# ogotoh/prrn_aln

Hardware: AMD Instinct MI355X
Metric: DP cells/s (profile-profile fwd2) + SP-score delta vs ref, 256x1024aa refinement (higher is better)
Workload: dtype f64; 1 GPU; prrn refinement sweep: 256 proteins x 1024 aa (seed 1), start MSA 5459 columns, 509 tree-branch divisions (HLF/RHF 256, GPF 253), 2.986e+09 in-band cells/sweep, band sh=-60; divisions=509, parallelism=divisions round-robin by size over 1 GPU(s), skeleton_corners=895772

## Files before the change

prrn_aln_amd/csrc/g2g_kernels.hip:

```cpp
#include <hip/hip_runtime.h>
#include <float.h>
#include <limits.h>
#include "g2g_device.h"

#define NEVSEL (-(DBL_MAX / 16 * 7))
#ifndef G2G_FWD_THREADS
#define G2G_FWD_THREADS 256
#endif
#ifndef G2G_V2_THREADS
#define G2G_V2_THREADS 256
#endif
#ifndef G2G_V2_MINWAVES
#define G2G_V2_MINWAVES 4
#endif
#ifndef G2G_V2_TILE_COLS
#define G2G_V2_TILE_COLS 256
#endif

enum { D_DEAD = 0, D_DIAG = 2, D_NEWD = 3, D_VERT = 4, D_HORI = 8, D_NEWV = 12, D_NEWH = 13 };
__device__ __forceinline__ bool isdiag(int d) { return d == D_DIAG || d == D_NEWD; }
__device__ __forceinline__ bool isvert(int d) { return d == D_VERT || d == D_NEWV; }
__device__ __forceinline__ bool ishori(int d) { return d == D_HORI || d == D_NEWH; }

enum { T_DIRMASK = 7, T_SEL2 = 8, T_GEXT = 16, T_G2EXT = 32, T_FEXT = 64, T_F2EXT = 128 };
// ... 61 lines not shown
    int k = 0;
    for (int di = 0; df.glen[di] >= 0; ++di) {
        while (df.glen[di] >= dld.glen(k + 1)) ++k;
        if (i < df.glen[di] + dld.nins(k)) break;
        g += df.freq[di];
    }
    return g;
}
__device__ __forceinline__ void cleardelta(const DList d) { d.set(0, 0, 0); d.set(1, INT_MAX, 0); }
__device__ void copydelta(const DList dst, const DList src)
{
    int k = 0;
    do { dst.set(k, src.glen(k), src.nins(k)); ++k; } while (src.glen(k) < INT_MAX);
    dst.set(k, src.glen(k), src.nins(k));
}
__device__ void newdelta(const DList dst, const SList df, const DList src)
{
    int kd = 0, ks = 0;
    int tg = 0, tn = 0;
    for (int di = 0; df.glen[di] >= 0; ++di) {
        int g = df.glen[di];
        if (g >= src.glen(ks)) {
            while (g >= src.glen(ks + 1)) ++ks;
            int sn = src.nins(ks);
            if (sn > tn) {
                dst.set(kd++, tg, tn);
                tn = sn;
                tg = g + 1;
            }
        }
    }
    dst.set(kd++, tg, tn);
    dst.set(kd, INT_MAX, 0);
}
__device__ void incdelta2(const DList dst, const DList src)
{
    int k = 0;
    do { dst.set(k, src.glen(k), src.nins(k) + 1); ++k; } while (src.glen(k) < INT_MAX);
    dst.set(k, src.glen(k), src.nins(k));
}

__device__ double sim2(const DevProb &P, int m, int n)
{
    const DevSide &a = P.a, &b = P.b;
    const uint8_t *ar = res_at(a, m), *br = res_at(b, n);
    const double *mtx = P.simmtx;
    const int dim = P.simdim;
    double s = 0;
    switch (P.sim2_kind) {
    case 0: return 0;
    case 11: return mtx[(size_t) ar[0] * dim + br[0]];
    case 120: for (int j = 0; j < b.many; ++j) s += mtx[(size_t) ar[0] * dim + br[j]]; return s;
    case 121: for (int j = 0; j < b.many; ++j) s += mtx[(size_t) ar[0] * dim + br[j]] * b.weight[j]; return s;
    case 13: return vss_at(b, n)[b.felm + ar[0]];
    case 210: for (int i = 0; i < a.many; ++i) s += mtx[(size_t) br[0] * dim + ar[i]]; return s;
    case 211: for (int i = 0; i < a.many; ++i) s += mtx[(size_t) br[0] * dim + ar[i]] * a.weight[i]; return s;
    case 220:
        for (int i = 0; i < a.many; ++i)
            for (int j = 0; j < b.many; ++j) s += mtx[(size_t) ar[i] * dim + br[j]];
        return s;
    case 221:
        for (int i = 0; i < a.many; ++i) {
            double st = 0;
            for (int j = 0; j < b.many; ++j) st += mtx[(size_t) ar[i] * dim + br[j]] * b.weight[j];
            s += st * a.weight[i];
        }
        return s;
    case 230: { const double *vb = vss_at(b, n) + b.felm;
        for (int i = 0; i < a.many; ++i) s += vb[ar[i]]; return s; }
    case 231: { const double *vb = vss_at(b, n) + b.felm;
        for (int i = 0; i < a.many; ++i) s += vb[ar[i]] * a.weight[i]; return s; }
    case 31: return vss_at(a, m)[a.felm + br[0]];
    case 320: { const double *va = vss_at(a, m) + a.felm;
        for (int j = 0; j < b.many; ++j) s += va[br[j]]; return s; }
    case 321: { const double *va = vss_at(a, m) + a.felm;
        for (int j = 0; j < b.many; ++j) s += va[br[j]] * b.weight[j]; return s; }
    case 33: { const double *va = vss_at(a, m) + a.felm, *vb = vss_at(b, n);
        for (int j = 0; j < b.felm; ++j) s += va[j] * vb[j]; return s; }
    case 330: { const double *va = vss_at(a, m) + a.felm, *vb = vss_at(b, n);
        const int dc[6] = {0, 1, 2, 3, 5, 9};
        for (int j = 0; j < b.felm; ++j) s += va[dc[j]] * vb[j]; return s; }
    }
    return 0;
}

__device__ __forceinline__ double unpa(const DevProb &P, int m, int n) { return thk_at(P.a, m)[0] * thk_at(P.b, n)[2] * -P.u; }
__device__ __forceinline__ double unpb(const DevProb &P, int n, int m) { return thk_at(P.b, n)[0] * thk_at(P.a, m)[2] * -P.u; }

__device__ double crg2(const DevProb &P, const int *gla, const int *glb, int st, int m, int n, int d3)
{
    const DevSide &a = P.a, &b = P.b;
    const uint8_t *as = res_at(a, m), *bs = res_at(b, n);
    const double *agd = a.gapdens + (size_t)(m + 1) * a.many, *apg = a.postgapdens + (size_t)(m + 1) * a.many;
    const double *bgd = b.gapdens + (size_t)(n + 1) * b.many, *bpg = b.postgapdens + (size_t)(n + 1) * b.many;
    const double *wa = a.weight, *wb = b.weight;
    const int an = a.many, bn = b.many;
#define GLA(i) gla[(size_t)(i) * st]
#define GLB(j) glb[(size_t)(j) * st]
#define NG(c) ((c) > 1)
    double g = 0;
    switch (P.crg2_kind) {
    case 11:
        if (d3 == 0) {
            if (NG(as[0]) && bgd[0] > 0 && GLA(0) >= GLB(0)) return bgd[0] * P.basic_gop;
            if (NG(bs[0]) && agd[0] > 0 && GLB(0) >= GLA(0)) return agd[0] * P.basic_gop;
        } else if (d3 > 0) {
            if (bpg[0] > 0 && GLA(0) >= GLB(0)) return bpg[0] * P.basic_gop;
        } else {
            if (apg[0] > 0 && GLB(0) >= GLA(0)) return apg[0] * P.basic_gop;
        }
        return 0;
    case 120: case 121: {
        const bool w = P.crg2_kind & 1;
        if (d3 == 0) {
            if (NG(as[0])) {
                for (int j = 0; j < bn; ++j) if (bgd[j] > 0 && GLA(0) >= GLB(j)) g += w ? wb[j] * bgd[j] : bgd[j];
            } else if (agd[0] > 0) {
                for (int j = 0; j < bn; ++j) if (NG(bs[j]) && GLB(j) >= GLA(0)) g += w ? wb[j] * agd[0] : agd[0];
            }
        } else if (d3 > 0) {
            if (NG(as[0]))
                for (int j = 0; j < bn; ++j) if (bpg[j] > 0 && GLA(0) >= GLB(j)) g += w ? wb[j] * bpg[j] : bpg[j];
        } else if (apg[0] > 0) {
            for (int j = 0; j < bn; ++j) if (NG(bs[j]) && GLB(j) >= GLA(0)) g += w ? wb[j] * apg[0] : apg[0];
        }
        return g * P.basic_gop;
    }
    case 210: case 211: {
        const bool w = P.crg2_kind & 1;
        if (d3 == 0) {
            if (NG(bs[0])) {
                for (int i = 0; i < an; ++i) if (agd[i] > 0 && GLB(0) >= GLA(i)) g += w ? wa[i] * agd[i] : agd[i];
            } else if (bgd[0] > 0) {
                for (int i = 0; i < an; ++i) if (NG(as[i]) && GLA(i) >= GLB(0)) g += w ? wa[i] * bgd[0] : bgd[0];
            }
        } else if (d3 < 0) {
            if (NG(bs[0]))
                for (int i = 0; i < an; ++i) if (apg[i] > 0 && GLB(0) >= GLA(i)) g += w ? wa[i] * apg[i] : apg[i];
        } else if (!w || (bs[0] && bs[1])) {
            if (bpg[0] > 0)
                for (int i = 0; i < an; ++i) if (NG(as[i]) && GLA(i) >= GLB(0)) g += w ? wa[i] * bpg[0] : bpg[0];
        }
        return g * P.basic_gop;
    }
    case 220:
        if (d3 == 0) {
            for (int i = 0; i < an; ++i) {
                if (NG(as[i])) {
                    for (int j = 0; j < bn; ++j) if (bgd[j] > 0 && GLA(i) >= GLB(j)) g += bgd[j];
                } else if (agd[i] > 0) {
                    for (int j = 0; j < bn; ++j) if (NG(bs[j]) && GLB(j) >= GLA(i)) g += agd[i];
                }
            }
        } else if (d3 > 0) {
            for (int i = 0; i < an; ++i)
                if (NG(as[i]))
                    for (int j = 0; j < bn; ++j) if (bpg[j] > 0 && GLA(i) >= GLB(j)) g += bpg[j];
        } else {
            for (int j = 0; j < bn; ++j)
                if (NG(bs[j]))
                    for (int i = 0; i < an; ++i) if (apg[i] > 0 && GLB(j) >= GLA(i)) g += apg[i];
        }
        return g * P.basic_gop;
    case 221:
        if (d3 == 0) {
            for (int i = 0; i < an; ++i) {
// ... 1342 lines not shown
```

prrn_aln_amd/csrc/g2g_kernels_v6.hip:

```cpp
#include <hip/hip_runtime.h>

#ifdef G2G_V6_STAMP
__device__ unsigned long long g2g_v6_stamp_acc[16];
#define V6_STAMP(k) { const unsigned long long t_ = __builtin_amdgcn_s_memtime(); st_acc[k] += t_ - st_t; st_t = t_; }
#define V6_STAMP_ARGS , unsigned long long (&st_acc)[12], unsigned long long &st_t
#define V6_STAMP_PASS , st_acc, st_t
#else
#define V6_STAMP(k)
#define V6_STAMP_ARGS
#define V6_STAMP_PASS
#endif

#include "g2g_lds.h"

struct LS6 { const lu32 *rows0; GLB unsigned *tw; int ia, ib; };
__device__ __forceinline__ GLB unsigned *ls6_twin(const LS6 &W, const lu32 *p, const int k) { return W.tw + 2 * (int) (p - W.rows0) + k; }
__device__ __forceinline__ unsigned ls6_rd(const LS6 &W, const lu32 *p, const int k, const int I) { return k < I ? p[k] : *ls6_twin(W, p, k); }
__device__ __forceinline__ void ls6_wr(const LS6 &W, lu32 *p, const int k, const int I, const unsigned v)
{
    if (k < I) p[k] = v;
    else { *ls6_twin(W, p, k) = v; asm volatile("s_waitcnt vmcnt(0)" ::: "memory"); }
}

#define V6_UNROLL _Pragma("clang loop unroll(full)")
// ... 472 lines not shown
            const GLB double *bfr = glb(b.freq[v]);
            lu32 *rk = (lu32 *) (lds + LO.ringk[v]);
            lf64 *rf = (lf64 *) (lds + LO.ringf[v]);
            const int S = v == 0 ? RS0 : RS1, base = v == 0 ? rbase0 : rbase1;
            for (int c0_ = fedcol + 1; c0_ <= upto; c0_ += 64) {
                const int col = c0_ + lane;
                if (col <= upto) {
                    const int k0 = bo[col + 1], len = bo[col + 2] - k0 - 1, c = k0 - (col + 1);
                    for (int e = 0; e < len; ++e) {
                        const int i = v6_ring_slot(c + e, base, S);
                        const unsigned key = v6_key(bgl[k0 + e]);
                        const double f = bfr[k0 + e];
                        rk[i] = key; rf[i] = f;
                        if (i < RT) { rk[S + i] = key; rf[S + i] = f; }
                    }
                }
            }
        }
        {
            const GLB double *bfr2 = glb(b.freq[2]);
            for (int c0_ = fedcol + 1; c0_ <= upto; c0_ += 64) {
                const int col = c0_ + lane;
                if (col <= upto) {
                    const int k2 = boff2[col + 1], lr_ = boff2[col + 2] - k2 - 1, lt_ = boff1[col + 2] - boff1[col + 1] - 1;
                    rhring[col & (V6_RHCOLS - 1)] = lr_ > lt_ ? bfr2[k2] : -1.;
                }
            }
        }
        if (upto > fedcol) fedcol = upto;
    };
    RS oH = rs_black(), oG = rs_black(), oG2 = rs_black(), oF = rs_black(), oF2 = rs_black();
    if (row_ok && m + 1 < a.right && m + 1 <= m_left_last && m + 1 + P.lw <= b.left) {
        lu32 *p = V6_L(lane + 1, SLOT_H(c0));
        const GLB unsigned *src = colH + (size_t) (m + 1 - a.left) * ndw;
        oH.val = __hiloint2double((int) V6_XLD(src + 1), (int) V6_XLD(src)); oH.dir = (int) V6_XLD(src + 2); oH.glb = (int) V6_XLD(src + 3);
        for (int k = 0; k < capa; ++k) { const unsigned v = V6_XLD(src + 4 + k); ls6_wr(W, p, k, ca4, v); if (v >= TERM) break; }
        for (int k = 0; k < capb; ++k) { const unsigned v = V6_XLD(src + 4 + capa + k); ls6_wr(W, p + ca4, k, cb4, v); if (v >= TERM) break; }
    }
    auto stage_load = [&](int col, bool wantG, unsigned &rh, unsigned &rg, unsigned &rg2) {
        if (lane < ndw) {
            const GLB unsigned *s = (col == b.left && vert0) ? colH + (size_t) (m0 - a.left) * ndw : rowHp + (size_t) col * ndw;
            rh = V6_XLD(s + lane);
            if (wantG) { rg = V6_XLD(rowGp + (size_t) col * ndw + lane); if (NOLL3) rg2 = V6_XLD(rowG2p + (size_t) col * ndw + lane); }
        }
    };
    auto stage_put = [&](int slot, int sid, unsigned v) {
        const int j = lane - 4;
        lu32 *const p = V6_L(0, slot);
        if (lane < 4) stsc[sid * 4 + lane] = v;
        else if (j < ca4 && j < capa) p[j] = v;
        else if (j >= capa && j - capa < cb4 && j < capa + capb) p[ca4 + j - capa] = v;
        if (capa > ca4 || capb > cb4) {
            const unsigned long long tb = __ballot(v >= TERM) >> 4;
            const int ta = tb ? (int) __builtin_ctzll(tb) : 63;
            const unsigned long long tbb = capa < 60 ? tb >> capa : 0ull;
            const int tbp = tbb ? (int) __builtin_ctzll(tbb) : 63;
            if (j >= ca4 && j < capa && j <= ta) ls6_wr(W, p, j, ca4, v);
            if (j >= capa + cb4 && j < capa + capb && j - capa <= tbp) ls6_wr(W, p + ca4, j - capa, cb4, v);
        }
    };
    auto stage_store = [&](int col, bool wantG, unsigned rh, unsigned rg, unsigned rg2) {
        if (lane < ndw) {
            stage_put(SLOT_H(col), SLOT_H(col), rh);
            if (wantG) { stage_put(SLOT_G(col), 3 + (col & 1), rg); if (NOLL3) stage_put(SLOT_G2(col), 5 + (col & 1), rg2); }
        }
    };
    StripSync S = strip_sync(prog_up, prog_self, dbg, failp, pgen, ti);
    if (lane < 28) stsc[lane] = 0;
    team_sync();
    refill(cbase);
    strip_need<V6Strip>(S, cbase + 1 <= c1 ? cbase + 1 : cbase);
    {
        unsigned rh = 0, rg = 0, rg2 = 0;
        stage_load(cbase, false, rh, rg, rg2);
        stage_store(cbase, false, rh, rg, rg2);
        if (cbase + 1 <= c1) {
            stage_load(cbase + 1, vert0, rh, rg, rg2);
            stage_store(cbase + 1, vert0, rh, rg, rg2);
        }
    }
    const double a_efq = row_ok ? thk_at(a, m)[2] : 0;
    const double pua_row = row_ok ? unpa(P, m, nlo) : 0;
    SimBlk SB; SB.buf = (GLBV3 double *) simscr; SB.cbase = cbase;
    simblk_fill(P, SB, 0, m0, lane);
    asm volatile("s_waitcnt vmcnt(0)" ::: "memory");
    double sim_cur = 0, bc_cur = 0;
    int os_cur = 0, oe_cur = 0, ot_cur = 0, te_cur = 0;
    bool have = false;
    RS hu = rs_black(), gu = rs_black(), g2u = rs_black(), hd;
    const bool do_vert = m > a.left;
    const bool wr_rows = mend < a.right;
    team_sync();
    unsigned st_h = 0, st_g = 0, st_g2 = 0;
    bool st_prev = false;
    bool p_act = false; int p_trb = 0; size_t p_tri = 0;
    const int ull = __builtin_amdgcn_readfirstlane(llast);
    int lhi = m0 + llast + P.up + 1; if (lhi > b.right) lhi = b.right;
    int llo = m0 + llast + P.lw; if (llo < b.left) llo = b.left;
    auto flush_rows = [&](const int nl) {
        if (nl >= llo && nl < lhi) {
            const int col = nl + 1;
            const int j = lane - 4;
#pragma unroll
            for (int x = 0; x < (NOLL3 ? 3 : 2); ++x) {
                const RS &r = (x == 0) ? oH : (x == 1) ? oG : oG2;
                const int slot = (x == 0) ? SLOT_H(col) : (x == 1) ? SLOT_G(col) : SLOT_G2(col);
                const unsigned v0 = (unsigned) __builtin_amdgcn_readlane(__double2loint(r.val), ull);
                const unsigned v1 = (unsigned) __builtin_amdgcn_readlane(__double2hiint(r.val), ull);
                const unsigned v2 = (unsigned) __builtin_amdgcn_readlane(r.dir, ull), v3 = (unsigned) __builtin_amdgcn_readlane(r.glb, ull);
                unsigned v = lane == 0 ? v0 : lane == 1 ? v1 : lane == 2 ? v2 : v3;
                if (lane >= 4 && lane < ndw) {
                    const lu32 *p = V6_L(llast + 1, slot);
                    v = (j < capa) ? (j < ca4 ? p[j] : TERM) : (j < capa + capb) ? (j - capa < cb4 ? p[ca4 + j - capa] : TERM) : 0;
                    if (capa > ca4 && p[ca4 - 1] < TERM && j >= ca4 && j < capa) v = ls6_rd(W, p, j, ca4);
                    if (capb > cb4 && p[ca4 + cb4 - 1] < TERM && j >= capa + cb4 && j < capa + capb) v = ls6_rd(W, p + ca4, j - capa, cb4);
                }
                GLB unsigned *dst = (x == 0) ? rowHc : (x == 1) ? rowGc : rowG2c;
                if (lane < ndw) V6_XST(dst + (size_t) col * ndw + lane, v);
            }
        }
    };
#ifdef G2G_V6_STAMP
    unsigned long long st_acc[12] = {0, 0, 0, 0, 0, 0, 0, 0, 0, 0, 0, 0};
    unsigned long long st_t = __builtin_amdgcn_s_memtime();
#endif
    strip_where(S);
    for (int s = 0; s < nsteps; ++s) {
        V6_STAMP(9)
        V6_BEAT(s)
        V6_MARK(1)
        const int n = cbase + s - lane;
        const int n0 = cbase + s;
        const bool active = row_ok && n >= lo && n < hi;
        if (st_prev) stage_store(n0 + 1, vert0, st_h, st_g, st_g2);
        if (p_act) trace[p_tri] = (uint8_t) p_trb;
        if (wr_rows && s > 0) flush_rows(n0 - 1 - llast);
        if (prog_self && s > 0 && (s & (pint - 1)) == 0) strip_publish<V6Strip>(S, n0 - llast);
        if ((s & (V6_FEED - 1)) == 0) { V6_MARK(2) refill(n0); team_sync(); }
        if ((s & 63) == 0) { V6_MARK(3) simblk_fill(P, SB, (s >> 6) + 1, m0, lane); asm volatile("s_waitcnt vmcnt(0)" ::: "memory"); }
        hd = hu;
        hu = rs_up(oH); gu = rs_up(oG);
        if (NOLL3) g2u = rs_up(oG2);
        strip_handover<V6Strip, NOLL3>(stsc, n0, lane, hd, hu, gu, g2u);
        double sim_nx = 0, bc_nx = 0;
        int os_nx = 0, oe_nx = 0, ot_nx = 0, te_nx = 0;
        if (active) {
            if (!have) {
                sim_cur = *simblk_at(SB, lane, n); bc_cur = bthk[(size_t) (n + 1) * 3];
                os_cur = boff0[n + 1]; oe_cur = boff0[n + 2]; ot_cur = boff1[n + 1]; te_cur = boff1[n + 2];
            }
            if (n + 1 < hi) {
                sim_nx = *simblk_at(SB, lane, n + 1); bc_nx = bthk[(size_t) (n + 2) * 3];
                os_nx = oe_cur; oe_nx = boff0[n + 3]; ot_nx = te_cur; te_nx = boff1[n + 3];
            }
        }
        st_prev = n0 + 1 < hi0 && n0 + 2 <= c1;
        if (st_prev) { V6_MARK(4) strip_need<V6Strip>(S, n0 + 2); stage_load(n0 + 2, vert0, st_h, st_g, st_g2); }
        V6_MARK(5)
        RS myH = oH, myG = oG, myG2 = oG2;
        V6_STAMP(0)
        if (active) {
            const bool do_hori = n > b.left;
            B6 B;
            B.rs = ring[0]; B.rt = ring[1];
            B.os = v6_ring_slot(os_cur - (n + 1), rbase0, RS0); B.ot = v6_ring_slot(ot_cur - (n + 1), rbase1, RS1);
            B.lens = oe_cur - os_cur - 1; B.lent = te_cur - ot_cur - 1;
            { const double hv = rhring[n & (V6_RHCOLS - 1)]; B.rhf = hv >= 0 ? hv : 0.; B.lenr = B.lent + (hv >= 0 ? 1 : 0); }
            const bool up_in = do_vert && (n - (m - 1) <= P.up);
            const bool left_in = (n - 1 - m >= P.lw);
            const RS bk = rs_black();
            const RS s_hu = rs_sel(up_in, hu, bk), s_gu = rs_sel(up_in, gu, bk), s_g2u = rs_sel(up_in, g2u, bk);
            const RS s_hl = rs_sel(left_in, oH, bk), s_fl = rs_sel(left_in, oF, bk), s_f2l = rs_sel(left_in, oF2, bk);
            const lu32 *hdl = V6_L(lane, SLOT_H(n));
            const lu32 *hul = up_in ? V6_L(lane, SLOT_H(n + 1)) : blk;
            const lu32 *gul = up_in ? V6_L(lane, SLOT_G(n + 1)) : blk;
            const lu32 *g2ul = (NOLL3 && up_in) ? V6_L(lane, SLOT_G2(n + 1)) : blk;
            const lu32 *hll = left_in ? V6_L(lane + 1, SLOT_H(n)) : blk;
            const lu32 *fll = left_in ? V6_L(lane + 1, SLOT_F) : blk;
            const lu32 *f2ll = (NOLL3 && left_in) ? V6_L(lane + 1, SLOT_F2) : blk;
            lu32 *const sink = (lu32 *) (lds + LO.sink) + lane;
            lu32 *const sink16 = (lu32 *) (lds + LO.sink) + 64 + 4 * lane;
            lu32 *dh = V6_L(lane + 1, SLOT_H(n + 1));
            lu32 *dg = V6_L(lane + 1, SLOT_G(n + 1));
            lu32 *dg2 = V6_L(lane + 1, NOLL3 ? SLOT_G2(n + 1) : SLOT_G(n + 1));
            lu32 *df = V6_L(lane + 1, SLOT_F);
            lu32 *df2 = V6_L(lane + 1, NOLL3 ? SLOT_F2 : SLOT_F);
            const double pua = a.nils ? unpa(P, m, n) : pua_row;
            const double pub = bc_cur * a_efq * -P.u;
            int trb = 0;
            if (!v6_cell_pf<NOLL3, NA, 5, false>(P, W, A, TAs, TAt, B, sink, sink16, hd, hdl, s_hu, hul, s_gu, gul, s_g2u, g2ul, s_hl, hll, s_fl, fll, s_f2l, f2ll,
                                  dh, dg, dg2, df, df2, do_vert, do_hori, sim_cur, pua, pub, myH, myG, myG2, oF, oF2, trb V6_STAMP_PASS))
                if (!v6_cell_pf<NOLL3, NA, 8, false>(P, W, A, TAs, TAt, B, sink, sink16, hd, hdl, s_hu, hul, s_gu, gul, s_g2u, g2ul, s_hl, hll, s_fl, fll, s_f2l, f2ll,
                                  dh, dg, dg2, df, df2, do_vert, do_hori, sim_cur, pua, pub, myH, myG, myG2, oF, oF2, trb V6_STAMP_PASS))
                    v6_cell_pf<NOLL3, NA, 8, true>(P, W, A, TAs, TAt, B, sink, sink16, hd, hdl, s_hu, hul, s_gu, gul, s_g2u, g2ul, s_hl, hll, s_fl, fll, s_f2l, f2ll,
                                  dh, dg, dg2, df, df2, do_vert, do_hori, sim_cur, pua, pub, myH, myG, myG2, oF, oF2, trb V6_STAMP_PASS);
            const int d = m + n;
            int mlo, mhi;
            diag_rows(d, a.left, a.right, b.left, b.right, P.lw, P.up, &mlo, &mhi);
            p_tri = (size_t) (d - P.d0) * P.tstride + (m - mlo);
            p_trb = trb;
            sim_cur = sim_nx; bc_cur = bc_nx; have = (n + 1 < hi);
            os_cur = os_nx; oe_cur = oe_nx; ot_cur = ot_nx; te_cur = te_nx;
            if (m == a.right - 1 && n == b.right - 1) *P.score = myH.val;
        }
        p_act = active;
        oH = myH; oG = myG; oG2 = myG2;
        V6_MARK(6)
        team_sync();
    }
    V6_MARK(7)
#ifdef G2G_V6_STAMP
    if (lane == 0) { for (int k = 0; k < 12; ++k) atomicAdd(&g2g_v6_stamp_acc[k], st_acc[k]); atomicAdd(&g2g_v6_stamp_acc[12], (unsigned long long) nsteps); }
#endif
    if (p_act) trace[p_tri] = (uint8_t) p_trb;
    if (wr_rows) flush_rows(cbase + nsteps - 1 - llast);
    strip_publish<V6Strip>(S, 0xFFFFF);
    V6_MARK(8)
#undef V6_L
}

#define V6_SIG(NAME, ATTR) extern "C" __global__ void ATTR                                         \
NAME(const DevProb *probs, const V2Tile *tiles, int ntiles, int *qhead, int *done, int gen, V6Lds LO, int pint, int pro_off, double *simscr, unsigned *twin, int twin_dw)
// ... 32 lines not shown
```

prrn_aln_amd/csrc/g2g_strip.h:

```cpp
#ifndef G2G_STRIP_H
#define G2G_STRIP_H

#define LDS __attribute__((address_space(3)))
typedef LDS char lchar;
typedef LDS unsigned lu32;
typedef LDS int li32;
typedef LDS double lf64;

#define GLB __attribute__((address_space(1)))
template <class T> __device__ __forceinline__ const GLB T *glb(const T *p) { return (const GLB T *) p; }
template <class T> __device__ __forceinline__ GLB T *glbw(T *p) { return (GLB T *) p; }

#define G2G_HDR 24
#include "g2g_lds.h"
#define G2G_DIAG 32
#ifdef G2G_POLL_RMW
#define G2G_POLL(p) __hip_atomic_fetch_or((int *) (p), 0, __ATOMIC_RELAXED, __HIP_MEMORY_SCOPE_AGENT)
#define G2G_POST(p, v) ((void) __hip_atomic_exchange((int *) (p), (int) (v), __ATOMIC_RELAXED, __HIP_MEMORY_SCOPE_AGENT))
#else
#define G2G_POLL(p) __hip_atomic_load((p), __ATOMIC_RELAXED, __HIP_MEMORY_SCOPE_AGENT)
#define G2G_POST(p, v) __hip_atomic_store((int *) (p), (int) (v), __ATOMIC_RELAXED, __HIP_MEMORY_SCOPE_AGENT)
#endif
#define G2G_GAP_TICKS 400000ull
__device__ __forceinline__ int g2g_wait_ge(const int *p, const int want, int *hdr, int *failp, const int slot)
// ... 108 lines not shown
#define G2G_RELEASE()
#else
#define G2G_XLD(p) (*(p))
#define G2G_XST(p, v) (*(p) = (v))
#define G2G_ACQUIRE() __builtin_amdgcn_fence(__ATOMIC_ACQUIRE, "agent")
#define G2G_RELEASE() __builtin_amdgcn_fence(__ATOMIC_RELEASE, "agent")
#endif
#ifdef G2G_HEARTBEAT
#define G2G_HB_STEP(pself, w, s) { if (pself) __hip_atomic_store((pself) + G2G_DIAG + 12 + 2 * (w), (int) (s), __ATOMIC_RELAXED, __HIP_MEMORY_SCOPE_AGENT); }
#define G2G_HB(pself, w, k) { if (pself) __hip_atomic_store((pself) + G2G_DIAG + 13 + 2 * (w), (int) (k), __ATOMIC_RELAXED, __HIP_MEMORY_SCOPE_AGENT); }
#else
#define G2G_HB_STEP(pself, w, s)
#define G2G_HB(pself, w, k)
#endif

__device__ __forceinline__ void team_sync()
{
    __builtin_amdgcn_fence(__ATOMIC_SEQ_CST, "wavefront");
    __builtin_amdgcn_wave_barrier();
}

__device__ __forceinline__ void chain_publish(int *prog, int penc, int v)
{
    asm volatile("s_waitcnt vmcnt(0)" ::: "memory");
    __builtin_amdgcn_fence(__ATOMIC_RELEASE, "agent");
    asm volatile("s_waitcnt vmcnt(0)" ::: "memory");
    G2G_POST(prog, penc | (v < 0xFFFFF ? v : 0xFFFFF));
}

__device__ __forceinline__ int uni(int x) { return __builtin_amdgcn_readfirstlane(x); }
__device__ __forceinline__ double uni(double x)
{
    return __hiloint2double(__builtin_amdgcn_readfirstlane(__double2hiint(x)), __builtin_amdgcn_readfirstlane(__double2loint(x)));
}
template <class T> __device__ __forceinline__ T *uni(T *p)
{
    const unsigned long long v = (unsigned long long) p;
    const unsigned lo = (unsigned) __builtin_amdgcn_readfirstlane((int) (unsigned) v);
    const unsigned hi = (unsigned) __builtin_amdgcn_readfirstlane((int) (unsigned) (v >> 32));
    return (T *) (((unsigned long long) hi << 32) | lo);
}
__device__ __forceinline__ void uni_side(DevSide &d, const DevSide &s)
{
    d.many = uni(s.many); d.len = uni(s.len); d.left = uni(s.left); d.right = uni(s.right); d.nils = uni(s.nils);
    d.nelm = uni(s.nelm); d.felm = uni(s.felm); d.hetero = uni(s.hetero); d.maxlist = uni(s.maxlist);
    d.seq = uni(s.seq); d.weight = uni(s.weight); d.pseq = uni(s.pseq); d.thk = uni(s.thk);
    for (int v = 0; v < 3; ++v) { d.off[v] = uni(s.off[v]); d.glen[v] = uni(s.glen[v]); d.freq[v] = uni(s.freq[v]); }
    d.gapdens = uni(s.gapdens); d.postgapdens = uni(s.postgapdens);
}
__device__ __forceinline__ void uni_prob(DevProb &d, const DevProb &s)
{
    d.kind = uni(s.kind); d.noll = uni(s.noll); d.sim2_kind = uni(s.sim2_kind); d.crg2_kind = uni(s.crg2_kind);
    d.codonk1 = uni(s.codonk1); d.lw = uni(s.lw); d.up = uni(s.up); d.width = uni(s.width);
    d.basic_gop = uni(s.basic_gop); d.weighted_gop = uni(s.weighted_gop); d.u = uni(s.u);
    d.u2divu1 = uni(s.u2divu1); d.v2divv1 = uni(s.v2divv1);
    d.simmtx = uni(s.simmtx); d.simdim = uni(s.simdim); d.capa = uni(s.capa); d.capb = uni(s.capb);
    uni_side(d.a, s.a); uni_side(d.b, s.b);
    d.v2_rowH = uni(s.v2_rowH); d.v2_rowG = uni(s.v2_rowG); d.v2_rowG2 = uni(s.v2_rowG2); d.v2_colH = uni(s.v2_colH);
    d.v2_cbH = uni(s.v2_cbH); d.v2_cbF = uni(s.v2_cbF); d.v2_cbF2 = uni(s.v2_cbF2);
    d.v2_rowstride = uni(s.v2_rowstride); d.v2_sim = uni(s.v2_sim); d.v2_rowoff = uni(s.v2_rowoff);
    d.trace = uni(s.trace); d.tstride = uni(s.tstride); d.d0 = uni(s.d0); d.d1 = uni(s.d1);
    d.score = uni(s.score);
}

#define GLBV3 __attribute__((address_space(1)))
#ifndef G2G_SIMBLK_STRIDE
#define G2G_SIMBLK_STRIDE (3 * 4096)
#endif
struct SimBlk { GLBV3 double *buf; int cbase; };
__device__ __forceinline__ void simblk_fill(const DevProb &P, const SimBlk &S, const int bk, const int m0, const int tid,
                                            const int nthr = 64, const int rows = 64)
{
    const int n = S.cbase + bk * 64 + (tid & 63);
    if (bk < 0 || n >= P.b.right) return;
    GLBV3 double *dst = S.buf + (size_t) (bk % 3) * 4096 + (tid & 63);
    for (int r = tid >> 6; r < rows; r += nthr >> 6) {
        const int m = m0 + r;
        if (m >= P.a.right) break;
        int nlo = m + P.lw; if (nlo < P.b.left) nlo = P.b.left;
        int nhi = m + P.up + 1; if (nhi > P.b.right) nhi = P.b.right;
        if (n >= nlo && n < nhi) dst[r * 64] = sim2(P, m, n);
    }
}
__device__ __forceinline__ const GLBV3 double *simblk_at(const SimBlk &S, const int row, const int n)
{
    const int k = n - S.cbase;
    return S.buf + (size_t) ((k >> 6) % 3) * 4096 + row * 64 + (k & 63);
}

struct RS { double val; int dir, glb; };
__device__ __forceinline__ RS rs_black() { RS r; r.val = NEVSEL; r.dir = 0; r.glb = 0; return r; }
__device__ __forceinline__ int dpp_up1(int x) { return __builtin_amdgcn_update_dpp(0, x, 0x138, 0xf, 0xf, false); }
__device__ __forceinline__ RS rs_up(const RS &x)
{
    RS r;
    r.val = __hiloint2double(dpp_up1(__double2hiint(x.val)), dpp_up1(__double2loint(x.val)));
    r.dir = dpp_up1(x.dir); r.glb = dpp_up1(x.glb);
    return r;
}
__device__ __forceinline__ RS rs_sel(bool c, const RS &x, const RS &y)
{
    RS r; r.val = c ? x.val : y.val; r.dir = c ? x.dir : y.dir; r.glb = c ? x.glb : y.glb; return r;
}

__device__ __forceinline__ int mod3(int c) { return ((c % 3) + 3) % 3; }
#define SLOT_H(c) (mod3(c))
#define SLOT_G(c) (3 + ((c) & 1))
#define SLOT_F 5
#define SLOT_G2(c) (6 + ((c) & 1))
#define SLOT_F2 8

struct StripTraits {
    static constexpr bool PUB_COL = false;
    static constexpr bool REC_GLB = true;
    static __device__ __forceinline__ void acquire() { __builtin_amdgcn_fence(__ATOMIC_ACQUIRE, "agent"); }
    static __device__ __forceinline__ void release() { __builtin_amdgcn_fence(__ATOMIC_RELEASE, "agent"); }
    static __device__ __forceinline__ void mark(int *, int) {}
};

struct StripSync { const int *prog_up; int *prog_self, *dbg, *failp; int penc, avail, ti; };
__device__ __forceinline__ StripSync strip_sync(const int *prog_up, int *prog_self, int *dbg, int *failp, const int pgen, const int ti)
{
    const StripSync S = {prog_up, prog_self, dbg, failp, (pgen & 0x7FF) << 20, prog_up ? 0 : 0x7fffffff, ti};
    return S;
}
template <class T>
__device__ __forceinline__ void strip_need(StripSync &S, const int col)
{
    const int want = S.penc | (col < 0xFFFFF ? col : 0xFFFFF);
    if (S.prog_up && want > S.avail) {
        S.avail = g2g_wait_ge(S.prog_up, want, S.dbg, S.failp, S.ti);
        T::acquire();
        asm volatile("s_waitcnt vmcnt(0)" ::: "memory");
    }
}
template <class T>
__device__ __forceinline__ void strip_publish(const StripSync &S, const int col)
{
    if (S.prog_self) {
        T::mark(S.prog_self, 9);
        asm volatile("s_waitcnt vmcnt(0)" ::: "memory");
        T::mark(S.prog_self, 10);
        T::release();
        asm volatile("s_waitcnt vmcnt(0)" ::: "memory");
        T::mark(S.prog_self, 11);
        if (T::PUB_COL) __hip_atomic_store(S.prog_self + G2G_DIAG + 8, col, __ATOMIC_RELAXED, __HIP_MEMORY_SCOPE_AGENT);
        G2G_POST(S.prog_self, S.penc | (col < 0 ? 0 : col < 0xFFFFF ? col : 0xFFFFF));
        T::mark(S.prog_self, 12);
    }
}
__device__ __forceinline__ void strip_where(const StripSync &S)
{
    if (S.prog_self) {
        __hip_atomic_store(S.prog_self + G2G_DIAG + 3, (int) __builtin_amdgcn_s_getreg((31 << 11) | 4), __ATOMIC_RELAXED, __HIP_MEMORY_SCOPE_AGENT);
        __hip_atomic_store(S.prog_self + G2G_DIAG + 4, 0x100 | ((int) __builtin_amdgcn_s_getreg((31 << 11) | 20) & 15), __ATOMIC_RELAXED, __HIP_MEMORY_SCOPE_AGENT);
    }
}

template <class T>
__device__ __forceinline__ RS strip_staged(const lu32 *q)
{
    RS t; t.val = *(const lf64 *) q; t.dir = (int) q[2]; t.glb = T::REC_GLB ? (int) q[3] : 0; return t;
}
template <class T, bool NOLL3>
__device__ __forceinline__ void strip_handover(const lu32 *stsc, const int n0, const int lane, RS &hd, RS &hu, RS &gu, RS &g2u)
{
// ... 30 lines not shown
```

Before: 5.707 billion cells/s.

## Compute similarity blocks cooperatively with per-kind wave-wide gather kernels

Replaces the per-cell generic sim2 call in the 64x64 similarity block prefill with specialised routines per sim2 kind. These load column residues and weights once per block and use readlane broadcasts to share row residue indices, profile vectors and weights across the wavefront, then gather matrix entries in batches of eight. The goal is to remove repeated per-cell index loads and branching, and to raise memory-level parallelism during the block refill inside the DP sweep. The cost is much more specialised code and register pressure, plus some risk from partial-count edge handling.

```diff
diff --git a/prrn_aln_amd/csrc/g2g_kernels.hip b/prrn_aln_amd/csrc/g2g_kernels.hip
--- a/prrn_aln_amd/csrc/g2g_kernels.hip
+++ b/prrn_aln_amd/csrc/g2g_kernels.hip
@@ -167,6 +167,233 @@
         for (int j = 0; j < b.felm; ++j) s += va[dc[j]] * vb[j]; return s; }
     }
     return 0;
+}
+
+#define SIMG __attribute__((address_space(1)))
+typedef const SIMG double *sb_dp;
+typedef const SIMG uint8_t *sb_bp;
+#define SB_G 8
+#define SB_CR 32
+#ifndef G2G_SIMBLK_VC
+#define G2G_SIMBLK_VC 24
+#endif
+struct SimRows {
+    SIMG double *dst; int n, nn, m0, r0, rstep, rows, lane;
+};
+__device__ __forceinline__ double sb_rl(double x, int l)
+{
+    return __hiloint2double(__builtin_amdgcn_readlane(__double2hiint(x), l), __builtin_amdgcn_readlane(__double2loint(x), l));
+}
+#define SB_KEEP(x) asm volatile("" : "+v"(x))
+__device__ __forceinline__ void sb_arrived(double (&x)[SB_G])
+{
+    static_assert(SB_G == 8, "sb_arrived names every element");
+    asm volatile("" : "+v"(x[0]), "+v"(x[1]), "+v"(x[2]), "+v"(x[3]), "+v"(x[4]), "+v"(x[5]), "+v"(x[6]), "+v"(x[7]));
+}
+__device__ __forceinline__ int sb_min(int x, int y) { return x < y ? x : y; }
+__device__ __forceinline__ void sb_store(const DevProb &P, const SimRows &R, int r, double s)
+{
+    const int m = R.m0 + r;
+    int nlo = m + P.lw; if (nlo < P.b.left) nlo = P.b.left;
+    int nhi = m + P.up + 1; if (nhi > P.b.right) nhi = P.b.right;
+    if (R.n >= nlo && R.n < nhi) R.dst[r * 64] = s;
+}
+__device__ __forceinline__ int sb_rows_res0(const DevProb &P, const SimRows &R)
+{
+    const int m = sb_min(R.m0 + R.lane, P.a.right - 1);
+    return ((sb_bp) P.a.seq)[(size_t) (m + 1) * P.a.many];
+}
+__device__ __forceinline__ void sb_col_res(const DevSide &b, const SimRows &R, int j0, int cnt, unsigned (&cr)[SB_CR / 4])
+{
+    const sb_bp br = (sb_bp) b.seq + (size_t) (R.nn + 1) * b.many + j0;
+#pragma unroll
+    for (int q = 0; q < SB_CR / SB_G; ++q) {
+        unsigned x[SB_G];
+        if (q * SB_G < cnt) {
+#pragma unroll
+            for (int t = 0; t < SB_G; ++t) x[t] = br[sb_min(q * SB_G + t, cnt - 1)];
+        } else {
+#pragma unroll
+            for (int t = 0; t < SB_G; ++t) x[t] = 0;
+        }
+#pragma unroll
+        for (int t = 0; t < SB_G; t += 4) cr[(q * SB_G + t) >> 2] = x[t] | (x[t + 1] << 8) | (x[t + 2] << 16) | (x[t + 3] << 24);
+    }
+}
+__device__ __forceinline__ double sb_lane_w(const double *w, const SimRows &R, int j0, int cnt)
+{
+    return ((sb_dp) w)[j0 + sb_min(R.lane, cnt - 1)];
+}
+template <bool W>
+__device__ __forceinline__ double sb_gather(const sb_dp base, const unsigned (&cr)[SB_CR / 4], const double wl, const int cnt, double s)
+{
+#pragma unroll
+    for (int q = 0; q < SB_CR / SB_G; ++q) {
+        if (q * SB_G < cnt) {
+            double x[SB_G];
+#pragma unroll
+            for (int t = 0; t < SB_G; ++t) { const int j = q * SB_G + t; x[t] = base[(cr[j >> 2] >> (8 * (j & 3))) & 255u]; }
+            sb_arrived(x);
+#pragma unroll
+            for (int t = 0; t < SB_G; ++t) {
+                const int j = q * SB_G + t;
+                if (j < cnt) { if (W) s += x[t] * sb_rl(wl, j); else s += x[t]; }
+            }
+        }
+    }
+    return s;
+}
+template <bool MTX, bool W>
+__device__ __forceinline__ void sb_by_colres(const DevProb &P, const SimRows &R)
+{
+    const DevSide &a = P.a, &b = P.b;
+    const int ar0 = MTX ? sb_rows_res0(P, R) : 0;
+    for (int j0 = 0; j0 < b.many; j0 += SB_CR) {
+        const int cnt = sb_min(SB_CR, b.many - j0);
+        unsigned cr[SB_CR / 4];
+        sb_col_res(b, R, j0, cnt, cr);
+        double wl = W ? sb_lane_w(b.weight, R, j0, cnt) : 0;
+        for (int r = R.r0; r < R.rows; r += R.rstep) {
+            const int m = R.m0 + r;
+            if (m >= a.right) break;
+            const sb_dp base = MTX ? (sb_dp) P.simmtx + (size_t) __builtin_amdgcn_readlane(ar0, r) * P.simdim
+                                   : (sb_dp) a.pseq + (size_t) (m + 1) * a.nelm + a.felm;
+            double s = 0;
+            if (j0) s = R.dst[r * 64];
+            SB_KEEP(wl);
+            s = sb_gather<W>(base, cr, wl, cnt, s);
+            sb_store(P, R, r, s);
+        }
+    }
+}
+template <bool MTX, bool W>
+__device__ __forceinline__ void sb_by_rowres(const DevProb &P, const SimRows &R)
+{
+    const DevSide &a = P.a, &b = P.b;
+    const sb_dp base = MTX ? (sb_dp) P.simmtx + (size_t) ((sb_bp) b.seq)[(size_t) (R.nn + 1) * b.many] * P.simdim
+                           : (sb_dp) b.pseq + (size_t) (R.nn + 1) * b.nelm + b.felm;
+    for (int i0 = 0; i0 < a.many; i0 += 64) {
+        const int cnt = sb_min(64, a.many - i0);
+        const int li = i0 + sb_min(R.lane, cnt - 1);
+        double wl = W ? sb_lane_w(a.weight, R, i0, cnt) : 0;
+        int ar_nx = ((sb_bp) a.seq)[(size_t) (sb_min(R.m0 + R.r0, a.right - 1) + 1) * a.many + li];
+        for (int r = R.r0; r < R.rows; r += R.rstep) {
+            const int m = R.m0 + r;
+            if (m >= a.right) break;
+            const int ar = ar_nx;
+            SB_KEEP(wl);
+            ar_nx = ((sb_bp) a.seq)[(size_t) (sb_min(m + R.rstep, a.right - 1) + 1) * a.many + li];
+            double s = 0;
+            if (i0) s = R.dst[r * 64];
+            for (int q = 0; q < cnt; q += SB_G) {
+                double x[SB_G];
+#pragma unroll
+                for (int t = 0; t < SB_G; ++t) x[t] = base[__builtin_amdgcn_readlane(ar, sb_min(q + t, cnt - 1))];
+                sb_arrived(x);
+#pragma unroll
+                for (int t = 0; t < SB_G; ++t)
+                    if (q + t < cnt) { if (W) s += x[t] * sb_rl(wl, q + t); else s += x[t]; }
+            }
+            sb_store(P, R, r, s);
+        }
+    }
+}
+template <bool W>
+__device__ __forceinline__ void sb_by_both(const DevProb &P, const SimRows &R)
+{
+    const DevSide &a = P.a, &b = P.b;
+    const bool held = b.many <= SB_CR;
+    unsigned cr[SB_CR / 4];
+    double wl = 0;
+    sb_col_res(b, R, 0, sb_min(SB_CR, b.many), cr);
+    if (W) wl = sb_lane_w(b.weight, R, 0, sb_min(SB_CR, b.many));
+    for (int r = R.r0; r < R.rows; r += R.rstep) {
+        const int m = R.m0 + r;
+        if (m >= a.right) break;
+        double s = 0;
+        SB_KEEP(wl);
+        for (int i0 = 0; i0 < a.many; i0 += 64) {
+            const int icnt = sb_min(64, a.many - i0);
+            const int ar = ((sb_bp) a.seq)[(size_t) (m + 1) * a.many + i0 + sb_min(R.lane, icnt - 1)];
+            const double wal = W ? sb_lane_w(a.weight, R, i0, icnt) : 0;
+            for (int i = 0; i < icnt; ++i) {
+                const sb_dp base = (sb_dp) P.simmtx + (size_t) __builtin_amdgcn_readlane(ar, i) * P.simdim;
+                double st = W ? 0 : s;
+                for (int j0 = 0; j0 < b.many; j0 += SB_CR) {
+                    const int cnt = sb_min(SB_CR, b.many - j0);
+                    if (!held) { sb_col_res(b, R, j0, cnt, cr); if (W) wl = sb_lane_w(b.weight, R, j0, cnt); }
+                    st = sb_gather<W>(base, cr, wl, cnt, st);
+                }
+                if (W) s += st * sb_rl(wal, i); else s = st;
+            }
+        }
+        sb_store(P, R, r, s);
+    }
+}
+template <bool DC>
+__device__ __forceinline__ void sb_by_vec(const DevProb &P, const SimRows &R)
+{
+    const DevSide &a = P.a, &b = P.b;
+    const sb_dp vb = (sb_dp) b.pseq + (size_t) (R.nn + 1) * b.nelm;
+    for (int j0 = 0; j0 < b.felm; j0 += G2G_SIMBLK_VC) {
+        const int cnt = sb_min(G2G_SIMBLK_VC, b.felm - j0);
+        double y[G2G_SIMBLK_VC];
+#pragma unroll
+        for (int t = 0; t < G2G_SIMBLK_VC; ++t) y[t] = vb[j0 + sb_min(t, cnt - 1)];
+        int lj = j0 + sb_min(R.lane, cnt - 1);
+        if (DC) lj = lj < 4 ? lj : lj == 4 ? 5 : 9;
+        double va_nx = ((sb_dp) a.pseq + (size_t) (sb_min(R.m0 + R.r0, a.right - 1) + 1) * a.nelm + a.felm)[lj];
+        for (int r = R.r0; r < R.rows; r += R.rstep) {
+            const int m = R.m0 + r;
+            if (m >= a.right) break;
+            const double va = va_nx;
+            va_nx = ((sb_dp) a.pseq + (size_t) (sb_min(m + R.rstep, a.right - 1) + 1) * a.nelm + a.felm)[lj];
+            double s = 0;
+            if (j0) s = R.dst[r * 64];
+#pragma unroll
+            for (int t = 0; t < G2G_SIMBLK_VC; ++t)
+                if (t < cnt) s += sb_rl(va, t) * y[t];
+            sb_store(P, R, r, s);
+        }
+    }
+}
+__device__ __forceinline__ void sb_by_one(const DevProb &P, const SimRows &R, const int kind)
+{
+    const DevSide &a = P.a, &b = P.b;
+    const int ar0 = (kind == 11 || kind == 13) ? sb_rows_res0(P, R) : 0;
+    const int br0 = (kind == 11 || kind == 31) ? ((sb_bp) b.seq)[(size_t) (R.nn + 1) * b.many] : 0;
+    const sb_dp vb = (sb_dp) b.pseq + (size_t) (R.nn + 1) * b.nelm + b.felm;
+    for (int r = R.r0; r < R.rows; r += R.rstep) {
+        const int m = R.m0 + r;
+        if (m >= a.right) break;
+        const int ar = __builtin_amdgcn_readlane(ar0, r);
+        double s = 0;
+        if (kind == 11) s = ((sb_dp) P.simmtx)[(size_t) ar * P.simdim + br0];
+        else if (kind == 13) s = vb[ar];
+        else if (kind == 31) s = ((sb_dp) a.pseq + (size_t) (m + 1) * a.nelm + a.felm)[br0];
+        sb_store(P, R, r, s);
+    }
+}
+__device__ __forceinline__ void sim2_block(const DevProb &P, const SimRows &R)
+{
+    switch (P.sim2_kind) {
+    case 120: sb_by_colres<true, false>(P, R); break;
+    case 121: sb_by_colres<true, true>(P, R); break;
+    case 320: sb_by_colres<false, false>(P, R); break;
+    case 321: sb_by_colres<false, true>(P, R); break;
+    case 210: sb_by_rowres<true, false>(P, R); break;
+    case 211: sb_by_rowres<true, true>(P, R); break;
+    case 230: sb_by_rowres<false, false>(P, R); break;
+    case 231: sb_by_rowres<false, true>(P, R); break;
+    case 220: sb_by_both<false>(P, R); break;
+    case 221: sb_by_both<true>(P, R); break;
+    case 33: sb_by_vec<false>(P, R); break;
+    case 330: sb_by_vec<true>(P, R); break;
+    case 11: sb_by_one(P, R, 11); break;
+    case 13: sb_by_one(P, R, 13); break;
+    case 31: sb_by_one(P, R, 31); break;
+    default: sb_by_one(P, R, 0); break;
+    }
 }
 
 __device__ __forceinline__ double unpa(const DevProb &P, int m, int n) { return thk_at(P.a, m)[0] * thk_at(P.b, n)[2] * -P.u; }
diff --git a/prrn_aln_amd/csrc/g2g_kernels_v6.hip b/prrn_aln_amd/csrc/g2g_kernels_v6.hip
--- a/prrn_aln_amd/csrc/g2g_kernels_v6.hip
+++ b/prrn_aln_amd/csrc/g2g_kernels_v6.hip
@@ -578,8 +578,6 @@
     const double a_efq = row_ok ? thk_at(a, m)[2] : 0;
     const double pua_row = row_ok ? unpa(P, m, nlo) : 0;
     SimBlk SB; SB.buf = (GLBV3 double *) simscr; SB.cbase = cbase;
-    simblk_fill(P, SB, 0, m0, lane);
-    asm volatile("s_waitcnt vmcnt(0)" ::: "memory");
     double sim_cur = 0, bc_cur = 0;
     int os_cur = 0, oe_cur = 0, ot_cur = 0, te_cur = 0;
     bool have = false;
@@ -633,7 +631,7 @@
         if (wr_rows && s > 0) flush_rows(n0 - 1 - llast);
         if (prog_self && s > 0 && (s & (pint - 1)) == 0) strip_publish<V6Strip>(S, n0 - llast);
         if ((s & (V6_FEED - 1)) == 0) { V6_MARK(2) refill(n0); team_sync(); }
-        if ((s & 63) == 0) { V6_MARK(3) simblk_fill(P, SB, (s >> 6) + 1, m0, lane); asm volatile("s_waitcnt vmcnt(0)" ::: "memory"); }
+        if ((s & 63) == 0) { V6_MARK(3) for (int bk = s ? (s >> 6) + 1 : 0; bk <= (s >> 6) + 1; ++bk) simblk_fill_block(P, SB, bk, m0, lane); asm volatile("s_waitcnt vmcnt(0)" ::: "memory"); }
         hd = hu;
         hu = rs_up(oH); gu = rs_up(oG);
         if (NOLL3) g2u = rs_up(oG2);
diff --git a/prrn_aln_amd/csrc/g2g_strip.h b/prrn_aln_amd/csrc/g2g_strip.h
--- a/prrn_aln_amd/csrc/g2g_strip.h
+++ b/prrn_aln_amd/csrc/g2g_strip.h
@@ -214,6 +214,21 @@
         if (n >= nlo && n < nhi) dst[r * 64] = sim2(P, m, n);
     }
 }
+__device__ __forceinline__ void simblk_fill_block(const DevProb &P, const SimBlk &S, const int bk, const int m0, const int tid,
+                                                  const int nthr = 64, const int rows = 64)
+{
+    const int n0 = S.cbase + bk * 64;
+    if (bk < 0 || n0 >= P.b.right) return;
+    SimRows R;
+    R.lane = tid & 63;
+    asm volatile("" : "+v"(R.lane));
+    R.n = n0 + R.lane; R.nn = R.n < P.b.right ? R.n : P.b.right - 1;
+    R.dst = S.buf + (size_t) (bk % 3) * 4096 + R.lane;
+    R.m0 = m0;
+    asm volatile("" : "+s"(R.m0));
+    R.r0 = __builtin_amdgcn_readfirstlane(tid >> 6); R.rstep = nthr >> 6; R.rows = rows;
+    sim2_block(P, R);
+}
 __device__ __forceinline__ const GLBV3 double *simblk_at(const SimBlk &S, const int row, const int n)
 {
     const int k = n - S.cbase;
```

Measured after the change: 5.832 billion cells/s, median of 6. 2.2% higher.
